# xin-fight/Research-and-Implementation-of-Image-Dehazing-Algorithm-Based-on-Vision-Transformer

Hardware: AMD Instinct MI355X
Metric: train patches/sec (128x128, embed_dim=32) (higher is better)
Workload: dtype f32; 1 GPU; Uformer_ProbSparse train step E=32 ps=128 per-GPU bs=32 fp32 Charbonnier+CR(VGG19, seeded-random weights) + AdamW (BASELINE configs[1]); global_batch=32, parallelism=dp1, arithmetic=fp32 storage/accumulate; products 6xbf16 MFMA, dropped <= 2^-24, split_terms=6

## Files before the change

### include/dehaze_hip.h

```cpp
#ifndef DEHAZE_HIP_H
#define DEHAZE_HIP_H

#include <stdint.h>

#ifdef __cplusplus
extern "C" {
#endif

#define DHZ_OK 0
#define DHZ_EINVAL (-22)
#define DHZ_ELAUNCH (-5)

#define DHZ_F32 0
#define DHZ_BF16 1

#define DHZ_NTOK 64
#define DHZ_NTOP 25

int dhz_abi_version(void);
const char* dhz_last_error(void);
const char* dhz_build_id(void);
int dhz_set_reserved_cus(int k);
int dhz_get_reserved_cus(void);
int dhz_grid_cus(void);
int dhz_set_deterministic(int on);
int dhz_get_deterministic(void);
int dhz_set_det_workspace(float* ws, size_t bytes);

int dhz_ps_attn_fwd(const float* q, const float* k, const float* v, int ld, const uint8_t* idx,
                    const float* bias, const float* mask, float* out, int ldo, uint8_t* rank,
                    int B_, int H, int nW, int d, void* stream);

int dhz_ps_attn_bwd_parts(int B_, int H);
int dhz_ps_attn_bwd_parts_d(int B_, int H, int d);
int dhz_ps_attn_bwd(const float* q, const float* k, const float* v, int ld, const float* bias,
                    const float* mask, const uint8_t* rank, const float* dout, int ldo, float* dq,
                    float* dk, float* dv, int ldg, float* dbias_part, int B_, int H, int nW, int d,
                    void* stream);

int dhz_fused_attn_prepack(const float* wq, const float* wk, const float* wv, const float* wo,
                           float* wqkv_p, float* wo_p, int C, void* stream);
int dhz_fused_attn_prepack_multi(const float* const* wq, const float* const* wk, const float* const* wv, const float* const* wo,
                                 float* const* wqkv_p, float* const* wo_p, const int* C, int n, void* stream);
int dhz_fused_window_attn_fwd(const float* x, const float* gamma, const float* beta, const float* wqkv_p,
                              const float* bqkv, const float* wo_p, const float* bo, const uint8_t* idx,
                              const float* bias, const float* mask, const float* drop_scale, float* out,
                              float* xn_save, float* qkv_save, float* ctx_save, float* stats_save,
                              uint8_t* rank_save, int B, int Hres, int Wres, int C, int shift,
                              void* stream);
int dhz_fused_window_attn_fwd6(const float* x, const float* gamma, const float* beta, const void* wqkv6_p, const float* bqkv,
                               const float* wo_p, const float* bo, const uint8_t* idx, const float* bias, const float* mask,
                               const float* drop_scale, float* out, float* xn_save, float* qkv_save, float* ctx_save, float* stats_save,
                               uint8_t* rank_save, int B, int Hres, int Wres, int C, int shift, void* stream);
// ... 304 lines not shown
```

### research-and-implementation-of-image-dehazing-algorithm-based-on-vision-transformer_amd/csrc/fused_attn.hip

```cpp
#include <stdlib.h>
#include "bf16_pipe.h"

namespace {

#ifndef FUSED_PERSIST_C32
#define FUSED_PERSIST_C32 1
#endif
#ifndef DHZ_FUSED_ABL
#define DHZ_FUSED_ABL 0
#endif
constexpr int NT = 64;
constexpr int NU = 25;
constexpr int SS = 68;
constexpr int HS = 36;

template <int CTRL>
__device__ __forceinline__ float dpp(float v) {
    return __int_as_float(__builtin_amdgcn_update_dpp(0, __float_as_int(v), CTRL, 0xF, 0xF, true));
}
__device__ __forceinline__ float r4max(float v) { v = fmaxf(v, dpp<0xB1>(v)); return fmaxf(v, dpp<0x4E>(v)); }
__device__ __forceinline__ float r4sum(float v) { v += dpp<0xB1>(v); return v + dpp<0x4E>(v); }
__device__ __forceinline__ float r8max(float v) { v = r4max(v); return fmaxf(v, dpp<0x141>(v)); }
__device__ __forceinline__ float r8sum(float v) { v = r4sum(v); return v + dpp<0x141>(v); }

// ... 20 lines not shown
    float vec[6 * C];
    int top[4][32];
    uint8_t idx[NT * NU];
};

template <int C, int SAVE, int NW = 1, bool P6 = false, bool PAD = false>
__global__ __launch_bounds__(256 * NW, NW == 2 ? 1 : (C == 64 ? 3 : (C == 128 ? 1 : 2))) void fused_window_attn_fwd_kernel(
    const float* __restrict__ x, const float* __restrict__ gamma, const float* __restrict__ beta,
    const float4* __restrict__ wqkv_p, const float* __restrict__ bqkv, const float4* __restrict__ wo_p,
    const float* __restrict__ bo, const uint8_t* __restrict__ idx, const float* __restrict__ bias,
    const float* __restrict__ mask, const float* __restrict__ dscale, float* __restrict__ out,
    float* __restrict__ xn_save, float* __restrict__ qkv_save, float* __restrict__ ctx_save,
    float* __restrict__ stats_save, uint8_t* __restrict__ rank_save, int Hres, int Wres, int shift, int nwin, PadArg<PAD> pad) {
    static_assert(!PAD || SAVE == 0, "padding words: inference instances only");
    constexpr int abl = DHZ_FUSED_ABL;
    constexpr int H = C / 32;
    constexpr int CPT = C / 4;
    constexpr int KS = C / 4;
    constexpr int KS4 = KS / 4;
    constexpr int P6_QKV_BYTES = (C / 32) * (C / 64 > 0 ? C / 64 : 1) * P6_RUNS * 1024;
    constexpr int P6O_RUNS = (C / 16) * 3;
    constexpr bool P6O = P6 && C >= 64 && P6O_RUNS * 1024 <= (int)sizeof(float) * NT * SS && P6O_RUNS % 4 == 0;
    extern __shared__ __attribute__((aligned(16))) unsigned char smem_raw[];
    const int half = NW == 2 ? (int)(threadIdx.x >> 8) : 0;
    FusedSmem<C>& sm = reinterpret_cast<FusedSmem<C>*>(smem_raw)[half];
    const int t = threadIdx.x & 255, lane = t & 63, w = t >> 6;
    const int i16 = lane & 15, g = lane >> 4;
    const int nWw = Wres >> 3, nW = (Hres >> 3) * nWw;
    const int tl = 16 * w + i16, qd = g;
    float* const P = sm.k;
// ... 58 lines not shown
            for (int i = 0; i < CPT / 4; ++i) {
                const float a0 = xv[i].x - mean, a1 = xv[i].y - mean, a2 = xv[i].z - mean, a3 = xv[i].w - mean;
                var += a0 * a0 + a1 * a1 + a2 * a2 + a3 * a3;
            }
            var = tok4sum(var);
            const float rstd = rsqrtf(var * (1.0f / C) + 1e-5f);
#pragma unroll
            for (int i = 0; i < CPT / 4; ++i) {
                const float4 gm = gmr[i], bt = btr[i];
                float4 y;
                y.x = (xv[i].x - mean) * rstd * gm.x + bt.x;
                y.y = (xv[i].y - mean) * rstd * gm.y + bt.y;
                y.z = (xv[i].z - mean) * rstd * gm.z + bt.z;
                y.w = (xv[i].w - mean) * rstd * gm.w + bt.w;
                xa[4 * i] = y.x; xa[4 * i + 1] = y.y; xa[4 * i + 2] = y.z; xa[4 * i + 3] = y.w;
                if (SAVE == 1 && !(abl & 128)) reinterpret_cast<float4*>(xn_save + ((size_t)win * NT + tl) * C + qd * CPT)[i] = y;
            }
            if (SAVE == 1 && !(abl & 128) && qd == 0) *reinterpret_cast<float2*>(stats_save + 2 * src_tok) = make_float2(mean, rstd);
        }
        dhz_u32x4 a6[P6 ? KS / 8 : 1][3];
        if constexpr (P6) {
#pragma unroll
            for (int kb = 0; kb < KS / 8; ++kb) dhz_split8x3(&xa[8 * kb], a6[kb][0], a6[kb][1], a6[kb][2]);
        }
        f32x4 oacc[C / 16];
#pragma unroll
        for (int i = 0; i < C / 16; ++i) oacc[i] = f32x4{0.f, 0.f, 0.f, 0.f};

#pragma unroll 1
        for (int h = 0; h < H; ++h) {
            if (!(abl & 1)) {
                const float (&a)[KS] = xa;
                f32x4 acc[6];
// ... 72 lines not shown
                        for (int j = 0; j < 6; ++j) acc[j] = mfma16(a[4 * s4 + 2], bc[j].z, acc[j]);
#pragma unroll
                        for (int j = 0; j < 6; ++j) acc[j] = mfma16(a[4 * s4 + 3], bc[j].w, acc[j]);
#pragma unroll
                        for (int j = 0; j < 6; ++j) bc[j] = bn[j];
                    }
                }
#pragma unroll
                for (int j = 0; j < 6; ++j) {
                    float* dst = (j < 2 ? sm.q : (j < 4 ? sm.k : sm.v)) + 16 * (j & 1) + i16;
#pragma unroll
                    for (int r = 0; r < 4; ++r) dst[(16 * w + 4 * g + r) * HS] = acc[j][r];
                }
            }
            __syncthreads();
            if (SAVE == 1 && !(abl & 128)) {
                const int row = t >> 2, c8 = (t & 3) * 8;
                float* dst = qkv_save + ((size_t)win * NT + row) * 3 * C + 32 * h + c8;
                *reinterpret_cast<float4*>(dst) = *reinterpret_cast<const float4*>(&sm.q[row * HS + c8]);
                *reinterpret_cast<float4*>(dst + 4) = *reinterpret_cast<const float4*>(&sm.q[row * HS + c8 + 4]);
                *reinterpret_cast<float4*>(dst + C) = *reinterpret_cast<const float4*>(&sm.k[row * HS + c8]);
                *reinterpret_cast<float4*>(dst + C + 4) = *reinterpret_cast<const float4*>(&sm.k[row * HS + c8 + 4]);
                *reinterpret_cast<float4*>(dst + 2 * C) = *reinterpret_cast<const float4*>(&sm.v[row * HS + c8]);
                *reinterpret_cast<float4*>(dst + 2 * C + 4) = *reinterpret_cast<const float4*>(&sm.v[row * HS + c8 + 4]);
            }
            if (!(abl & 2)) {
                float a[8], kb[4][8];
                f32x4 sacc[4];
                ld4(&sm.q[(16 * w + i16) * HS + 8 * g], &a[0]);
                ld4(&sm.q[(16 * w + i16) * HS + 8 * g + 4], &a[4]);
#pragma unroll
// ... 439 lines not shown
    DHZ_CHECK_LAUNCH("dhz_fused_attn_prepack_multi");
    return DHZ_OK;
}

static int fused_fwd_impl(bool p6, const float* x, const float* gamma, const float* beta, const float* wqkv_p,
                          const float* bqkv, const float* wo_p, const float* bo, const uint8_t* idx,
                          const float* bias, const float* mask, const float* drop_scale, float* out,
                          float* xn_save, float* qkv_save, float* ctx_save, float* stats_save,
                          uint8_t* rank_save, int B, int Hres, int Wres, int C, int shift, void* stream, const uint64_t* pad = nullptr) {
    DHZ_REQUIRE(x && gamma && beta && wqkv_p && bqkv && wo_p && bo && idx && out, "dhz_fused_window_attn_fwd: null pointer");
    DHZ_REQUIRE(C == 32 || C == 64 || C == 128, "dhz_fused_window_attn_fwd: C=%d unsupported (32, 64, 128)", C);
    DHZ_REQUIRE(B > 0 && Hres % 8 == 0 && Wres % 8 == 0 && Hres >= 8 && Wres >= 8 && shift >= 0 && shift < 8,
                "dhz_fused_window_attn_fwd: bad geometry %dx%d shift %d", Hres, Wres, shift);
    const bool any4 = xn_save || qkv_save || ctx_save || stats_save;
    const bool all4 = xn_save && qkv_save && ctx_save && stats_save;
    DHZ_REQUIRE(!any4 || (all4 && rank_save),
                "dhz_fused_window_attn_fwd: save buffers: none, rank_save alone, or all five");
    const int save = all4 ? 1 : (rank_save ? 2 : 0);
    DHZ_REQUIRE(!mask || shift > 0, "dhz_fused_window_attn_fwd: a mask is only meaningful for shifted windows");
    hipStream_t s = (hipStream_t)stream;
    const int nwin = B * (Hres / 8) * (Wres / 8);
#define GO(CC)                                                                                                      \
    do {                                                                                                            \
        if (save == 1) launch_fused<CC, 1>(s, nwin, x, gamma, beta, wqkv_p, bqkv, wo_p, bo, idx, bias, mask, drop_scale, \
                                           out, xn_save, qkv_save, ctx_save, stats_save, rank_save, Hres, Wres, shift);   \
        else if (save == 2) launch_fused<CC, 2>(s, nwin, x, gamma, beta, wqkv_p, bqkv, wo_p, bo, idx, bias, mask, drop_scale, \
                                                out, nullptr, nullptr, nullptr, nullptr, rank_save, Hres, Wres, shift);      \
        else if (pad) launch_fused<CC, 0, 1, false, true>(s, nwin, x, gamma, beta, wqkv_p, bqkv, wo_p, bo, idx, bias, mask, drop_scale, out, \
                                                          nullptr, nullptr, nullptr, nullptr, nullptr, Hres, Wres, shift, pad); \
        else launch_fused<CC, 0>(s, nwin, x, gamma, beta, wqkv_p, bqkv, wo_p, bo, idx, bias, mask, drop_scale, out, \
                                 nullptr, nullptr, nullptr, nullptr, nullptr, Hres, Wres, shift);                \
    } while (0)
#ifdef DHZ_DIAG
    static const int pair_env = getenv("DHZ_FUSED_PAIR") ? atoi(getenv("DHZ_FUSED_PAIR")) : 0;
#else
    constexpr int pair_env = 0;
#endif
    if (C == 64 && pair_env == 2 && nwin % 2 == 0 && !pad) {
        if (save == 1) launch_fused<64, 1, 2>(s, nwin, x, gamma, beta, wqkv_p, bqkv, wo_p, bo, idx, bias, mask, drop_scale, out, xn_save,
                                              qkv_save, ctx_save, stats_save, rank_save, Hres, Wres, shift);
        else if (save == 2) launch_fused<64, 2, 2>(s, nwin, x, gamma, beta, wqkv_p, bqkv, wo_p, bo, idx, bias, mask, drop_scale, out,
                                                   nullptr, nullptr, nullptr, nullptr, rank_save, Hres, Wres, shift);
        else launch_fused<64, 0, 2>(s, nwin, x, gamma, beta, wqkv_p, bqkv, wo_p, bo, idx, bias, mask, drop_scale, out, nullptr, nullptr,
                                    nullptr, nullptr, nullptr, Hres, Wres, shift);
    } else if (p6) {
        DHZ_REQUIRE(C == 32 || C == 64 || C == 128, "dhz_fused_window_attn_fwd6: C=%d unsupported (32, 64, 128)", C);
#define GO6(CC)                                                                                                             \
    do {                                                                                                                    \
        if (save == 1) launch_fused<CC, 1, 1, true>(s, nwin, x, gamma, beta, wqkv_p, bqkv, wo_p, bo, idx, bias, mask, drop_scale, out, xn_save, \
                                                    qkv_save, ctx_save, stats_save, rank_save, Hres, Wres, shift);         \
        else if (save == 2) launch_fused<CC, 2, 1, true>(s, nwin, x, gamma, beta, wqkv_p, bqkv, wo_p, bo, idx, bias, mask, drop_scale, out, \
                                                         nullptr, nullptr, nullptr, nullptr, rank_save, Hres, Wres, shift); \
        else if (pad) launch_fused<CC, 0, 1, true, true>(s, nwin, x, gamma, beta, wqkv_p, bqkv, wo_p, bo, idx, bias, mask, drop_scale, out, nullptr, \
                                                         nullptr, nullptr, nullptr, nullptr, Hres, Wres, shift, pad);      \
        else launch_fused<CC, 0, 1, true>(s, nwin, x, gamma, beta, wqkv_p, bqkv, wo_p, bo, idx, bias, mask, drop_scale, out, nullptr, nullptr, \
                                          nullptr, nullptr, nullptr, Hres, Wres, shift);                                   \
    } while (0)
        if (C == 32) GO6(32); else if (C == 64) GO6(64); else GO6(128);
#undef GO6
    } else if (C == 32) GO(32); else if (C == 64) GO(64); else GO(128);
#undef GO
    DHZ_CHECK_LAUNCH("dhz_fused_window_attn_fwd");
    return DHZ_OK;
}

extern "C" int dhz_fused_attn_prepack6_multi(const float* const* wq, const float* const* wk, const float* const* wv, const float* const* wo,
                                             void* const* wqkv6_p, const int* C, int n, void* stream) {
// ... 51 lines not shown
```

### research-and-implementation-of-image-dehazing-algorithm-based-on-vision-transformer_amd/csrc/ps_attn.hip

```cpp
#include "bf16_pipe.h"

namespace {

constexpr int NT = 64;
constexpr int NU = 25;
constexpr int SS = 68;

#ifndef PSF_WG32
#define PSF_WG32 3
#endif
#ifndef PSF_WG64
#define PSF_WG64 3
#endif

__device__ __forceinline__ dhz_bf16x8 frag_bf16(const float* row, int half, int g) {
    const f32x4 lo = *reinterpret_cast<const f32x4*>(row + 32 * half + 8 * g);
    const f32x4 hi = *reinterpret_cast<const f32x4*>(row + 32 * half + 8 * g + 4);
    dhz_u32x4 r;
    r[0] = dhz_pack_top(lo[1], lo[0]); r[1] = dhz_pack_top(lo[3], lo[2]);
    r[2] = dhz_pack_top(hi[1], hi[0]); r[3] = dhz_pack_top(hi[3], hi[2]);
    return __builtin_bit_cast(dhz_bf16x8, r);
}
__device__ __forceinline__ f32x4 tile_mma_bf16_k64(const float* A, int lda, const float* B, int ldb, int i16, int g, f32x4 acc) {
    acc = __builtin_amdgcn_mfma_f32_16x16x32_bf16(frag_bf16(A + i16 * lda, 0, g), frag_bf16(B + i16 * ldb, 0, g), acc, 0, 0, 0);
// ... 487 lines not shown
                if (r < NU) val = *reinterpret_cast<const float4*>(&dqs[r * DS + c4 * 4]);
                st4(dq + go, val);
            }
        }
    }

    if (HAS_BIAS && REG_ACC) {
        float* dst = dbias_part + (size_t)blockIdx.x * NT * NT;
#pragma unroll
        for (int i = 0; i < 16; ++i) dst[(w + 4 * i) * NT + lane] = accr[i];
    }
    if (HAS_BIAS && !REG_ACC) {
        __syncthreads();
        float4* dst = reinterpret_cast<float4*>(dbias_part + (size_t)blockIdx.x * NT * NT);
        for (int e = t; e < NT * NT / 4; e += 256) dst[e] = reinterpret_cast<const float4*>(sm.acc)[e];
    }
}

__global__ void bias_gather_kernel(const float* __restrict__ table, float* __restrict__ bias, int H) {
    const int e = blockIdx.x * blockDim.x + threadIdx.x;
    if (e >= H * NT * NT) return;
    const int h = e / (NT * NT), i = (e / NT) % NT, j = e % NT;
    const int rel = ((i >> 3) - (j >> 3) + 7) * 15 + ((i & 7) - (j & 7) + 7);
    bias[e] = table[rel * H + h];
}

constexpr int BIAS_MULTI_MAX = 32;
struct BiasMulti { const float* table[BIAS_MULTI_MAX]; float* bias[BIAS_MULTI_MAX]; int H[BIAS_MULTI_MAX]; };
__global__ void bias_gather_multi_kernel(const BiasMulti d) {
    const int H = d.H[blockIdx.y];
// ... 223 lines not shown
    dhz_set_error("dhz_ps_attn_bwd_dt: unknown dtype %d", dtype);
    return DHZ_EINVAL;
}
extern "C" int dhz_ps_attn_bwd_dt_pad(const void* q, const void* k, const void* v, int ld, const float* bias,
                                      const float* mask, const uint64_t* pad, const uint8_t* rank, const void* dout, int ldo, void* dq,
                                      void* dk, void* dv, int ldg, float* dbias_part, int B_, int H, int nW, int d,
                                      int dtype, void* stream) {
    DHZ_REQUIRE_PAD("dhz_ps_attn_bwd_dt_pad");
    if (dtype == DHZ_F32) return ps_attn_bwd_t<float>((const float*)q, (const float*)k, (const float*)v, ld, bias, mask, rank, (const float*)dout, ldo, (float*)dq, (float*)dk, (float*)dv, ldg, dbias_part, B_, H, nW, d, stream, pad);
    if (dtype == DHZ_BF16) return ps_attn_bwd_t<bf16s>((const bf16s*)q, (const bf16s*)k, (const bf16s*)v, ld, bias, mask, rank, (const bf16s*)dout, ldo, (bf16s*)dq, (bf16s*)dk, (bf16s*)dv, ldg, dbias_part, B_, H, nW, d, stream, pad);
    dhz_set_error("dhz_ps_attn_bwd_dt_pad: unknown dtype %d", dtype);
    return DHZ_EINVAL;
}
#undef DHZ_REQUIRE_PAD

extern "C" int dhz_bias_gather(const float* table, float* bias, int H, void* stream) {
    DHZ_REQUIRE(table && bias && H > 0, "dhz_bias_gather: bad arguments");
    const int n = H * NT * NT;
    hipLaunchKernelGGL(bias_gather_kernel, dim3((n + 255) / 256), dim3(256), 0, (hipStream_t)stream, table, bias, H);
    DHZ_CHECK_LAUNCH("dhz_bias_gather");
    return DHZ_OK;
}

extern "C" int dhz_bias_gather_multi(const float* const* tables, float* const* biases, const int* heads, int n, void* stream) {
    DHZ_REQUIRE(tables && biases && heads && n > 0 && n <= BIAS_MULTI_MAX, "dhz_bias_gather_multi: null pointer or n=%d outside 1..%d", n,
                BIAS_MULTI_MAX);
    BiasMulti d = {};
    int hmax = 0;
    for (int i = 0; i < n; ++i) {
        DHZ_REQUIRE(tables[i] && biases[i] && heads[i] > 0, "dhz_bias_gather_multi: entry %d: null pointer or H=%d", i, heads[i]);
// ... 63 lines not shown
```

### research-and-implementation-of-image-dehazing-algorithm-based-on-vision-transformer_amd/dehaze_hip/_lib.py

```python
import ctypes
import os

_HERE = os.path.dirname(os.path.abspath(__file__))
LIB_PATH = os.environ.get("DHZ_LIB_PATH") or os.path.join(_HERE, "libdehaze_hip.so")

c_f = ctypes.c_void_p
c_p = ctypes.c_void_p
c_i = ctypes.c_int
c_l = ctypes.c_int64
c_fl = ctypes.c_float

SIGNATURES = {
    "dhz_abi_version": [],
    "dhz_last_error": [],
    "dhz_build_id": [],
    "dhz_set_reserved_cus": [ctypes.c_int],
    "dhz_gelu_fwd_dt": [ctypes.c_void_p, ctypes.c_void_p, ctypes.c_int64, ctypes.c_int, ctypes.c_void_p],
    "dhz_gelu_bwd_dt": [ctypes.c_void_p, ctypes.c_void_p, ctypes.c_void_p, ctypes.c_int64, ctypes.c_void_p, ctypes.c_int64, ctypes.c_int, ctypes.c_void_p],
    "dhz_get_reserved_cus": [],
    "dhz_set_deterministic": [ctypes.c_int],
    "dhz_get_deterministic": [],
    "dhz_set_det_workspace": [ctypes.c_void_p, ctypes.c_size_t],
    "dhz_grid_cus": [],
    "dhz_ps_attn_fwd": [c_f, c_f, c_f, c_i, c_p, c_f, c_f, c_f, c_i, c_p, c_i, c_i, c_i, c_i, c_p],
    "dhz_ps_attn_bwd_parts": [c_i, c_i],
    "dhz_ps_attn_bwd_parts_d": [c_i, c_i, c_i],
    "dhz_ps_attn_bwd": [c_f, c_f, c_f, c_i, c_f, c_f, c_p, c_f, c_i, c_f, c_f, c_f, c_i, c_f, c_i, c_i, c_i, c_i, c_p],
    "dhz_fused_attn_prepack": [c_f, c_f, c_f, c_f, c_f, c_f, c_i, c_p],
    "dhz_fused_window_attn_fwd": [c_f, c_f, c_f, c_f, c_f, c_f, c_f, c_p, c_f, c_f, c_f, c_f, c_f, c_f, c_f, c_f, c_p,
                                  c_i, c_i, c_i, c_i, c_i, c_p],
    "dhz_fused_window_attn_fwd6": [c_f, c_f, c_f, c_f, c_f, c_f, c_f, c_p, c_f, c_f, c_f, c_f, c_f, c_f, c_f, c_f, c_p,
                                   c_i, c_i, c_i, c_i, c_i, c_p],
    "dhz_fused_attn_prepack6": [c_f, c_f, c_f, c_f, c_p, c_i, c_p],
    "dhz_fused_attn_prepack6_multi": [c_p, c_p, c_p, c_p, c_p, c_p, c_i, c_p],
    "dhz_fused_attn_bwd_parts": [c_i],
    "dhz_fused_attn_bwd_prepack": [c_f, c_f, c_f, c_f, c_f, c_i, c_p],
    "dhz_fused_window_attn_bwd": [c_f] * 11 + [c_f] * 12 + [c_i, c_i, c_i, c_i, c_i, c_p],
    "dhz_dense_attn_fwd": [c_f, c_f, c_f, c_i, c_f, c_f, c_f, c_i, c_i, c_i, c_i, c_i, c_fl, c_p],
    "dhz_dense_attn_bwd": [c_f, c_f, c_f, c_i, c_f, c_f, c_f, c_i, c_f, c_f, c_f, c_i, c_f, c_i, c_i, c_i, c_i, c_fl, c_p],
    "dhz_bias_gather": [c_f, c_f, c_i, c_p],
    "dhz_bias_gather_multi": [c_p, c_p, c_p, c_i, c_p],
    "dhz_fused_attn_prepack_multi": [c_p, c_p, c_p, c_p, c_p, c_p, c_p, c_i, c_p],
# ... 172 lines not shown
```

### research-and-implementation-of-image-dehazing-algorithm-based-on-vision-transformer_amd/dehaze_hip/fused.py

```python
import torch
from torch.autograd import Function

from . import _lib, ops
from .ops import NTOK, _grad_buf, _int_array, _p, _ptr_array, _ready, _require_gpu, _stream

SUPPORTED_C = (32, 64, 128)
ENABLED = True
ATTN_FUSED_C128_MAX_HW = int(__import__("os").environ.get("DHZ_FUSED_C128_MAX_HW", "1024"))
ATTN_FUSED_BWD_C = (32,)


def _fused_bwd_widths():
    return () if ops.DETERMINISTIC else ATTN_FUSED_BWD_C
ATTN_FUSED_P6 = __import__("os").environ.get("DHZ_FUSED_P6", "1") != "0"
ATTN_FUSED_P6_C = (64, 128)
ATTN_FUSED_PAD_P6_C = (64, 128)
LEFF_FUSED = True
LEFF_FUSED_C = (32, 64)
LEFF_FUSED_C64_MAX_T = 262144
LEFF_FUSED_P6 = __import__("os").environ.get("DHZ_LEFF_P6", "1") != "0"
LEFF_FUSED_P6_C = (64,)
LEFF_BWD_DZ = __import__("os").environ.get("DHZ_LEFF_BWD_DZ", "1") != "0"
LEFF_BWD_DZ_C = (32, 64, 128)


def _wgrad(dy, off, x, w, b, row_scale=None):
    return ops.linear_wgrad(dy, off, x, [(w, b)], row_scale)


def _ln_backward(dxn, x, gamma_p, beta_p, gamma, stats, dres, B, Hres, Wres, C, shift, partition, dres_windowed=False, dx_window=None,
                 dx2=None):
    dx = torch.empty_like(x)
    gg, gb = _grad_buf(gamma_p), _grad_buf(beta_p)
    lay = (1 if dres_windowed else 0, 0 if dx_window is None else 1, 0 if dx_window is None else int(dx_window))
    d2 = None
    if dx2 is not None:
        d2 = torch.empty_like(x)
        lay = (lay[0], lay[1], int(dx2[0]))
# ... 154 lines not shown
            _lib.call("dhz_fused_attn_prepack", _p(wq), _p(wk), _p(wv), _p(wo), _p(wqkv_p), _p(wo_p), C, _stream())
    wqkv_f32 = wqkv_p
    if use6:
        hit = STAGED_PACK6.pop(id(wq), None)
        if hit is not None and hit[0] is wq and hit[1].numel() == n6 and hit[1].device == dev:
            wqkv_p = hit[1]
        else:
            wqkv_p = torch.empty(n6, device=dev, dtype=torch.bfloat16)
            _lib.call("dhz_fused_attn_prepack6", _p(wq), _p(wk), _p(wv), _p(wo), _p(wqkv_p), C, _stream())
        if wo_p is None:
            wo_p = wqkv_p
    bqkv = ops.cat_rows([bq.detach(), bk.detach(), bv.detach()])
    bias = _bias_tile(table, H, dev)
    out = torch.empty_like(x)
    fused_bwd = train and C in _fused_bwd_widths() and x.dtype == torch.float32
    xn = qkv = cx = stats = rank = None
    if train:
        if not fused_bwd:
            xn = torch.empty((T, C), **f32)
            qkv = torch.empty((T, 3 * C), **f32)
            cx = torch.empty((T, C), **f32)
            stats = torch.empty((T, 2), **f32)
        rank = torch.empty(((T // NTOK) * H * NTOK,), device=dev, dtype=torch.uint8)
    entry = "dhz_fused_window_attn_fwd6" if use6 else "dhz_fused_window_attn_fwd"
    ev = ops._timed("dhz_fused_window_attn_fwd")
    if pad is not None:
        assert pad.is_cuda and pad.dtype == torch.int64 and pad.numel() == T // NTOK and pad.is_contiguous(), \
            f"padding words {tuple(pad.shape)} {pad.dtype} on {pad.device}"
        _lib.call("dhz_fused_window_attn_fwd_pad", 1 if use6 else 0, _p(x), _p(gamma), _p(beta), _p(wqkv_p), _p(bqkv), _p(wo_p), _p(bo), _p(idx),
                  _p(bias), _p(mask), _p(pad), _p(dscale), _p(out), B, Hres, Wres, C, shift, _stream())
    else:
        _lib.call(entry, _p(x), _p(gamma), _p(beta), _p(wqkv_p), _p(bqkv), _p(wo_p), _p(bo), _p(idx),
                  _p(bias), _p(mask), _p(dscale), _p(out), _p(xn), _p(qkv), _p(cx), _p(stats), _p(rank), B, Hres, Wres, C,
                  shift, _stream())
    ops._timed_end(ev, T // NTOK, C)
    rec = None
# ... 62 lines not shown


def _attn_bwd(rec, dout, windowed=False, daw_pre=None):
    if rec.kind == "attn_fused_bwd":
        assert not windowed
        return _attn_bwd_fused(rec, dout)
    x, gamma, stats, xn, qkv, cx, rank, bias, mask, dscale, wq_, wk_, wv_, wo_ = rec.saved
    wq, bq, wk, bk, wv, bv, wo, bo, gamma_p, beta_p, table_p = rec.params
    B, Hres, Wres, C, shift, H = rec.geom
    d = C // H
    dout = dout.contiguous()
    dev = x.device
    T = B * Hres * Wres
    B_ = T // NTOK
    f32 = dict(device=dev, dtype=torch.float32)
    if daw_pre is not None:
        daw = daw_pre.view(T, C)
        dctx = ops.gemm_dgrad(daw, wo_)
        g_wo, g_bo = _wgrad(daw, 0, cx, wo, bo)
    elif windowed:
        daw = dout.view(T, C)
        rs = (dscale, Hres * Wres) if dscale is not None else None
        dctx = ops.gemm_dgrad(daw, wo_, rs)
        g_wo, g_bo = _wgrad(daw, 0, cx, wo, bo, rs)
    else:
        daw = torch.empty((T, C), device=dev, dtype=dout.dtype)
        _lib.call("dhz_reverse_residual_bwd_dt", _p(dout), _p(dscale), _p(daw), B, Hres, Wres, C, shift, 1, ops._dt(dout), _stream())
        dctx = ops.gemm_dgrad(daw, wo_)
        g_wo, g_bo = _wgrad(daw, 0, cx, wo, bo)
    dqkv = torch.empty_like(qkv)
    parts = _lib.load().dhz_ps_attn_bwd_parts_d(B_, H, d)
    dpart = torch.empty((parts, NTOK, NTOK), **f32) if bias is not None else None
    ops.ps_attn_bwd_launch(qkv, dqkv, bias, mask, rank, dctx, dpart, B_, H, d)
    dtable = _table_backward(dpart, parts, table_p, H, dev) if bias is not None else None
    dxn, (g_wq, g_bq, g_wk, g_bk, g_wv, g_bv) = ops.linear_bwd_pair(dqkv, xn, ops.cat_rows([wq_.detach(), wk_.detach(), wv_.detach()]),
                                                                    [(wq, bq), (wk, bk), (wv, bv)])
    dx, dgamma, dbeta = _ln_backward(dxn, x, gamma_p, beta_p, gamma, stats, dout, B, Hres, Wres, C, shift, 1, dres_windowed=windowed)
    return (dx, dgamma, dbeta, g_wq, g_bq, g_wk, g_bk, g_wv, g_bv, g_wo, g_bo, dtable)


def fused_c128_ok(HW):
    return HW <= ATTN_FUSED_C128_MAX_HW or not torch.is_grad_enabled()


def use_fused_attn(C, dtype, heads, HW):
    return ENABLED and dtype == torch.float32 and C == 32 * heads and (C in (32, 64) or (C == 128 and fused_c128_ok(HW)))


# ... 261 lines not shown
```

Before: 1034 patches/s.

## Fuse attention out-projection backward into ProbSparse attention backward kernel

Adds a ProbSparse attention backward kernel that also does the out-projection backward. It computes dctx from daw and Wo inside the kernel, accumulates dWo/dbo with fp32 atomics, and exploits the rank structure so that only the top rows plus one mean row of daw are needed. The forward then no longer saves the ctx buffer for C=64 (new save mode 3). This removes a separate dgrad GEMM, a wgrad GEMM and a T×C ctx write and read. The trade-offs are atomic contention on the weight gradients, no support for deterministic mode, and the path only runs for C=64 layers.

```diff
diff --git a/include/dehaze_hip.h b/include/dehaze_hip.h
--- a/include/dehaze_hip.h
+++ b/include/dehaze_hip.h
@@ -37,6 +37,11 @@
                     const float* mask, const uint8_t* rank, const float* dout, int ldo, float* dq,
                     float* dk, float* dv, int ldg, float* dbias_part, int B_, int H, int nW, int d,
                     void* stream);
+
+int dhz_ps_attn_bwd_outproj(const float* q, const float* k, const float* v, int ld, const float* bias, const float* mask,
+                            const uint8_t* rank, const float* daw, int lda, const float* wo, const float* row_scale, int wins_per_scale,
+                            float* dq, float* dk, float* dv, int ldg, float* dbias_part, float* dwo, float* dbo, int B_, int H, int nW,
+                            int d, void* stream);
 
 int dhz_fused_attn_prepack(const float* wq, const float* wk, const float* wv, const float* wo,
                            float* wqkv_p, float* wo_p, int C, void* stream);
diff --git a/research-and-implementation-of-image-dehazing-algorithm-based-on-vision-transformer_amd/csrc/fused_attn.hip b/research-and-implementation-of-image-dehazing-algorithm-based-on-vision-transformer_amd/csrc/fused_attn.hip
--- a/research-and-implementation-of-image-dehazing-algorithm-based-on-vision-transformer_amd/csrc/fused_attn.hip
+++ b/research-and-implementation-of-image-dehazing-algorithm-based-on-vision-transformer_amd/csrc/fused_attn.hip
@@ -58,6 +58,7 @@
     float* __restrict__ stats_save, uint8_t* __restrict__ rank_save, int Hres, int Wres, int shift, int nwin, PadArg<PAD> pad) {
     static_assert(!PAD || SAVE == 0, "padding words: inference instances only");
     constexpr int abl = DHZ_FUSED_ABL;
+    constexpr bool SAVE_CHAIN = SAVE == 1 || SAVE == 3;
     constexpr int H = C / 32;
     constexpr int CPT = C / 4;
     constexpr int KS = C / 4;
@@ -146,9 +147,9 @@
                 y.z = (xv[i].z - mean) * rstd * gm.z + bt.z;
                 y.w = (xv[i].w - mean) * rstd * gm.w + bt.w;
                 xa[4 * i] = y.x; xa[4 * i + 1] = y.y; xa[4 * i + 2] = y.z; xa[4 * i + 3] = y.w;
-                if (SAVE == 1 && !(abl & 128)) reinterpret_cast<float4*>(xn_save + ((size_t)win * NT + tl) * C + qd * CPT)[i] = y;
-            }
-            if (SAVE == 1 && !(abl & 128) && qd == 0) *reinterpret_cast<float2*>(stats_save + 2 * src_tok) = make_float2(mean, rstd);
+                if (SAVE_CHAIN && !(abl & 128)) reinterpret_cast<float4*>(xn_save + ((size_t)win * NT + tl) * C + qd * CPT)[i] = y;
+            }
+            if (SAVE_CHAIN && !(abl & 128) && qd == 0) *reinterpret_cast<float2*>(stats_save + 2 * src_tok) = make_float2(mean, rstd);
         }
         dhz_u32x4 a6[P6 ? KS / 8 : 1][3];
         if constexpr (P6) {
@@ -251,7 +252,7 @@
                 }
             }
             __syncthreads();
-            if (SAVE == 1 && !(abl & 128)) {
+            if (SAVE_CHAIN && !(abl & 128)) {
                 const int row = t >> 2, c8 = (t & 3) * 8;
                 float* dst = qkv_save + ((size_t)win * NT + row) * 3 * C + 32 * h + c8;
                 *reinterpret_cast<float4*>(dst) = *reinterpret_cast<const float4*>(&sm.q[row * HS + c8]);
@@ -721,9 +722,10 @@
                 "dhz_fused_window_attn_fwd: bad geometry %dx%d shift %d", Hres, Wres, shift);
     const bool any4 = xn_save || qkv_save || ctx_save || stats_save;
     const bool all4 = xn_save && qkv_save && ctx_save && stats_save;
-    DHZ_REQUIRE(!any4 || (all4 && rank_save),
-                "dhz_fused_window_attn_fwd: save buffers: none, rank_save alone, or all five");
-    const int save = all4 ? 1 : (rank_save ? 2 : 0);
+    const bool no_ctx = xn_save && qkv_save && !ctx_save && stats_save && C != 32;
+    DHZ_REQUIRE(!any4 || ((all4 || no_ctx) && rank_save),
+                "dhz_fused_window_attn_fwd: save buffers: none, rank_save alone, all five, or (C = 64 / 128) all but ctx_save");
+    const int save = all4 ? 1 : (no_ctx ? 3 : (rank_save ? 2 : 0));
     DHZ_REQUIRE(!mask || shift > 0, "dhz_fused_window_attn_fwd: a mask is only meaningful for shifted windows");
     hipStream_t s = (hipStream_t)stream;
     const int nwin = B * (Hres / 8) * (Wres / 8);
@@ -733,6 +735,8 @@
                                            out, xn_save, qkv_save, ctx_save, stats_save, rank_save, Hres, Wres, shift);   \
         else if (save == 2) launch_fused<CC, 2>(s, nwin, x, gamma, beta, wqkv_p, bqkv, wo_p, bo, idx, bias, mask, drop_scale, \
                                                 out, nullptr, nullptr, nullptr, nullptr, rank_save, Hres, Wres, shift);      \
+        else if (save == 3) { if constexpr (CC != 32) launch_fused<CC, 3>(s, nwin, x, gamma, beta, wqkv_p, bqkv, wo_p, bo, idx, bias, mask, drop_scale, \
+                                                out, xn_save, qkv_save, nullptr, stats_save, rank_save, Hres, Wres, shift); }  \
         else if (pad) launch_fused<CC, 0, 1, false, true>(s, nwin, x, gamma, beta, wqkv_p, bqkv, wo_p, bo, idx, bias, mask, drop_scale, out, \
                                                           nullptr, nullptr, nullptr, nullptr, nullptr, Hres, Wres, shift, pad); \
         else launch_fused<CC, 0>(s, nwin, x, gamma, beta, wqkv_p, bqkv, wo_p, bo, idx, bias, mask, drop_scale, out, \
@@ -743,7 +747,7 @@
 #else
     constexpr int pair_env = 0;
 #endif
-    if (C == 64 && pair_env == 2 && nwin % 2 == 0 && !pad) {
+    if (C == 64 && pair_env == 2 && nwin % 2 == 0 && !pad && save != 3) {
         if (save == 1) launch_fused<64, 1, 2>(s, nwin, x, gamma, beta, wqkv_p, bqkv, wo_p, bo, idx, bias, mask, drop_scale, out, xn_save,
                                               qkv_save, ctx_save, stats_save, rank_save, Hres, Wres, shift);
         else if (save == 2) launch_fused<64, 2, 2>(s, nwin, x, gamma, beta, wqkv_p, bqkv, wo_p, bo, idx, bias, mask, drop_scale, out,
@@ -758,6 +762,8 @@
                                                     qkv_save, ctx_save, stats_save, rank_save, Hres, Wres, shift);         \
         else if (save == 2) launch_fused<CC, 2, 1, true>(s, nwin, x, gamma, beta, wqkv_p, bqkv, wo_p, bo, idx, bias, mask, drop_scale, out, \
                                                          nullptr, nullptr, nullptr, nullptr, rank_save, Hres, Wres, shift); \
+        else if (save == 3) { if constexpr (CC != 32) launch_fused<CC, 3, 1, true>(s, nwin, x, gamma, beta, wqkv_p, bqkv, wo_p, bo, idx, bias, mask, drop_scale, out, \
+                                                         xn_save, qkv_save, nullptr, stats_save, rank_save, Hres, Wres, shift); } \
         else if (pad) launch_fused<CC, 0, 1, true, true>(s, nwin, x, gamma, beta, wqkv_p, bqkv, wo_p, bo, idx, bias, mask, drop_scale, out, nullptr, \
                                                          nullptr, nullptr, nullptr, nullptr, Hres, Wres, shift, pad);      \
         else launch_fused<CC, 0, 1, true>(s, nwin, x, gamma, beta, wqkv_p, bqkv, wo_p, bo, idx, bias, mask, drop_scale, out, nullptr, nullptr, \
diff --git a/research-and-implementation-of-image-dehazing-algorithm-based-on-vision-transformer_amd/csrc/ps_attn.hip b/research-and-implementation-of-image-dehazing-algorithm-based-on-vision-transformer_amd/csrc/ps_attn.hip
--- a/research-and-implementation-of-image-dehazing-algorithm-based-on-vision-transformer_amd/csrc/ps_attn.hip
+++ b/research-and-implementation-of-image-dehazing-algorithm-based-on-vision-transformer_amd/csrc/ps_attn.hip
@@ -525,6 +525,280 @@
         __syncthreads();
         float4* dst = reinterpret_cast<float4*>(dbias_part + (size_t)blockIdx.x * NT * NT);
         for (int e = t; e < NT * NT / 4; e += 256) dst[e] = reinterpret_cast<const float4*>(sm.acc)[e];
+    }
+}
+
+template <int C>
+struct OutprojSmem {
+    static constexpr int CS = C + 4;
+    BwdSmem<32> core;
+    float tile[32 * CS];
+};
+static_assert(sizeof(BwdSmem<32>) % 16 == 0, "the daw tile starts 16-byte aligned");
+
+template <int C, bool HAS_BIAS>
+__global__ __launch_bounds__(256) void ps_attn_bwd_outproj_kernel(
+    const float* __restrict__ q, const float* __restrict__ k, const float* __restrict__ v, int ld,
+    const float* __restrict__ bias, const float* __restrict__ mask, const uint8_t* __restrict__ rank_in,
+    const float* __restrict__ daw, int lda, const float* __restrict__ wo, const float* __restrict__ row_scale, int wins_per_scale,
+    float* __restrict__ dq, float* __restrict__ dk, float* __restrict__ dv, int ldg, float* __restrict__ dbias_part,
+    float* __restrict__ dwo, float* __restrict__ dbo, int B_, int nW) {
+    constexpr int D = 32, H = C / 32;
+    constexpr int DS = D + 4, CS = C + 4;
+    constexpr int F = D / 4, RPP = 256 / F, NR = NT / RPP;
+    constexpr int FC = C / 4, RC = 256 / FC, NRC = NT / RC;
+    constexpr int NW = C / 32;
+    extern __shared__ __attribute__((aligned(16))) unsigned char smem_raw[];
+    OutprojSmem<C>& so = *reinterpret_cast<OutprojSmem<C>*>(smem_raw);
+    BwdSmem<D>& sm = so.core;
+    float* const tile = so.tile;
+    const int t = threadIdx.x, lane = t & 63, w = t >> 6;
+    const int i16 = lane & 15, g = lane >> 4;
+    const int bid = blockIdx.x;
+    const int h = bid % H;
+    const int bstep = gridDim.x / H;
+    const float scale = rsqrtf((float)D);
+    const int tr = w & 1, tc2 = w >> 1;
+
+    if (HAS_BIAS) {
+        for (int e = t; e < NT * NT / 4; e += 256) reinterpret_cast<float4*>(sm.acc)[e] = make_float4(0.f, 0.f, 0.f, 0.f);
+    }
+    float wf[C / 4];
+#pragma unroll
+    for (int s = 0; s < C / 4; ++s) wf[s] = wo[(size_t)(4 * s + g) * C + 32 * h + 16 * tc2 + i16];
+    f32x4 accw[NW];
+#pragma unroll
+    for (int ii = 0; ii < NW; ++ii) accw[ii] = f32x4{0.f, 0.f, 0.f, 0.f};
+    float dbacc = 0.f;
+
+    f32x4 pk[NR], pv[NR], pq[NR], pg[NRC];
+    uint8_t prank = 255;
+    auto prefetch = [&](int b) {
+        const size_t tok0 = (size_t)b * NT;
+        const int c4 = t % F;
+#pragma unroll
+        for (int p = 0; p < NR; ++p) {
+            const size_t gi = (tok0 + p * RPP + t / F) * ld + h * D + c4 * 4;
+            pk[p] = ld4v(k + gi);
+            pv[p] = ld4v(v + gi);
+            pq[p] = ld4v(q + gi);
+        }
+#pragma unroll
+        for (int p = 0; p < NRC; ++p) pg[p] = ld4v(daw + (tok0 + p * RC + t / FC) * lda + (t % FC) * 4);
+        if (t < NT) prank = rank_in[((size_t)b * H + h) * NT + t];
+    };
+    if (bid / H < B_) prefetch(bid / H);
+
+    for (int b = bid / H; b < B_; b += bstep) {
+        const size_t tok0 = (size_t)b * NT;
+        const float rs = row_scale ? row_scale[b / wins_per_scale] : 1.0f;
+        __syncthreads();
+        if (t < NT) {
+            const uint8_t r = prank;
+            sm.rank[t] = r;
+            if (r < NU) sm.top[r] = t;
+        } else if (t < NT + 32 - NU) {
+            sm.top[NU + t - NT] = 0;
+        }
+        for (int e = t; e < (32 - NU) * DS; e += 256) sm.qr[NU * DS + e] = 0.f;
+        for (int e = t; e < (31 - NU) * CS; e += 256) tile[(NU + 1) * CS + e] = 0.f;
+        __syncthreads();
+
+        {
+            const int c4 = t % F;
+#pragma unroll
+            for (int p = 0; p < NR; ++p) {
+                const int row = p * RPP + t / F;
+                *reinterpret_cast<f32x4*>(&sm.k[row * DS + c4 * 4]) = pk[p];
+                *reinterpret_cast<f32x4*>(&sm.v[row * DS + c4 * 4]) = pv[p];
+                const int r = sm.rank[row];
+                if (r < NU) *reinterpret_cast<f32x4*>(&sm.qr[r * DS + c4 * 4]) = pq[p];
+            }
+            const int cc = t % FC;
+            f32x4 dm = {0.f, 0.f, 0.f, 0.f};
+#pragma unroll
+            for (int p = 0; p < NRC; ++p) {
+                const int r = sm.rank[p * RC + t / FC];
+                const f32x4 val = pg[p] * rs;
+                if (r < NU) *reinterpret_cast<f32x4*>(&tile[r * CS + cc * 4]) = val;
+                else dm += val;
+            }
+            if (b + bstep < B_) prefetch(b + bstep);
+#pragma unroll
+            for (int o = FC; o < 64; o <<= 1) {
+                dm[0] += __shfl_xor(dm[0], o); dm[1] += __shfl_xor(dm[1], o);
+                dm[2] += __shfl_xor(dm[2], o); dm[3] += __shfl_xor(dm[3], o);
+            }
+            if (lane < FC) *reinterpret_cast<f32x4*>(&sm.ds[w * C + lane * 4]) = dm;
+        }
+        __syncthreads();
+        if (t < C) tile[NU * CS + t] = sm.ds[t] + sm.ds[C + t] + sm.ds[2 * C + t] + sm.ds[3 * C + t];
+
+        {
+#pragma unroll
+            for (int ii = 0; ii < 2; ++ii) {
+                const int tc = (w >> 1) + 2 * ii;
+                f32x4 acc = {0.f, 0.f, 0.f, 0.f};
+                acc = tile_mma<D / 4>(sm.qr + 16 * tr * DS, DS, 1, sm.k + 16 * tc * DS, DS, 1, acc);
+#pragma unroll
+                for (int j = 0; j < 4; ++j) sm.p1[(16 * tr + 4 * g + j) * SS + 16 * tc + i16] = acc[j];
+            }
+        }
+        __syncthreads();
+
+        {
+            f32x4 acc = {0.f, 0.f, 0.f, 0.f};
+            const float* ap = tile + (16 * tr + i16) * CS + g;
+#pragma unroll
+            for (int s = 0; s < C / 4; ++s) acc = mfma16(ap[4 * s], wf[s], acc);
+#pragma unroll
+            for (int j = 0; j < 4; ++j) sm.dor[(16 * tr + 4 * g + j) * DS + 16 * tc2 + i16] = acc[j];
+        }
+        {
+            const int r = t >> 3, c0 = (t & 7) * 8;
+            float p1[8], p2[8];
+            if (r < NU) {
+                const int qrow = sm.top[r];
+                float x[8];
+#pragma unroll
+                for (int i = 0; i < 8; ++i) x[i] = sm.p1[r * SS + c0 + i] * scale;
+                const float* brow = bias ? bias + ((size_t)h * NT + qrow) * NT + c0 : nullptr;
+                const float* mrow = mask ? mask + ((size_t)(b % nW) * NT + qrow) * NT + c0 : nullptr;
+                double_softmax8<false>(x, brow, mrow, p1, p2);
+            } else {
+                const float f = (r == NU) ? (1.0f / NT) : 0.f;
+#pragma unroll
+                for (int i = 0; i < 8; ++i) { p1[i] = 0.f; p2[i] = f; }
+            }
+#pragma unroll
+            for (int i = 0; i < 8; ++i) { sm.p1[r * SS + c0 + i] = p1[i]; sm.p2[r * SS + c0 + i] = p2[i]; }
+        }
+        __syncthreads();
+
+        f32x4 accv[D / 16];
+        f32x4 accp[2];
+        f32x4 acco = {0.f, 0.f, 0.f, 0.f};
+        {
+#pragma unroll
+            for (int tc = 0; tc < D / 16; ++tc) {
+                f32x4 acc = {0.f, 0.f, 0.f, 0.f};
+                accv[tc] = tile_mma<8>(sm.p2 + 16 * w, 1, SS, sm.dor + 16 * tc, 1, DS, acc);
+            }
+#pragma unroll
+            for (int ii = 0; ii < 2; ++ii) {
+                const int tc = (w >> 1) + 2 * ii;
+                f32x4 acc = {0.f, 0.f, 0.f, 0.f};
+                accp[ii] = tile_mma<D / 4>(sm.dor + 16 * tr * DS, DS, 1, sm.v + 16 * tc * DS, DS, 1, acc);
+            }
+            acco = tile_mma<16>(sm.p2 + 16 * tr * SS, SS, 1, sm.v + 16 * tc2, 1, DS, acco);
+        }
+        __syncthreads();
+        {
+#pragma unroll
+            for (int tc = 0; tc < D / 16; ++tc)
+#pragma unroll
+                for (int j = 0; j < 4; ++j) sm.v[(16 * w + 4 * g + j) * DS + 16 * tc + i16] = accv[tc][j];
+#pragma unroll
+            for (int ii = 0; ii < 2; ++ii) {
+                const int tc = (w >> 1) + 2 * ii;
+#pragma unroll
+                for (int j = 0; j < 4; ++j) sm.ds[(16 * tr + 4 * g + j) * SS + 16 * tc + i16] = accp[ii][j];
+            }
+#pragma unroll
+            for (int j = 0; j < 4; ++j) sm.dor[(16 * tr + 4 * g + j) * DS + 16 * tc2 + i16] = acco[j];
+        }
+        __syncthreads();
+
+        {
+            const int r = t >> 3, c0 = (t & 7) * 8;
+            float dp[8], p1[8], p2[8];
+            float dot2 = 0.f;
+#pragma unroll
+            for (int i = 0; i < 8; ++i) {
+                dp[i] = sm.ds[r * SS + c0 + i]; p1[i] = sm.p1[r * SS + c0 + i]; p2[i] = sm.p2[r * SS + c0 + i];
+                dot2 += dp[i] * p2[i];
+            }
+            dot2 = dhz_row8_sum(dot2);
+            float da[8], dot1 = 0.f;
+#pragma unroll
+            for (int i = 0; i < 8; ++i) { da[i] = p2[i] * (dp[i] - dot2); dot1 += da[i] * p1[i]; }
+            dot1 = dhz_row8_sum(dot1);
+            if (HAS_BIAS && r < NU) {
+                float* arow = sm.acc + sm.top[r] * NT + c0;
+#pragma unroll
+                for (int i = 0; i < 8; ++i) arow[i] += da[i];
+            }
+#pragma unroll
+            for (int i = 0; i < 8; ++i) sm.ds[r * SS + c0 + i] = p1[i] * (da[i] - dot1) * scale;
+
+            const int c4 = t % F;
+#pragma unroll
+            for (int p = 0; p < NR; ++p) {
+                const int row = p * RPP + t / F;
+                st4(dv + (tok0 + row) * ldg + h * D + c4 * 4, *reinterpret_cast<const float4*>(&sm.v[row * DS + c4 * 4]));
+            }
+        }
+        __syncthreads();
+
+        f32x4 accq;
+        f32x4 acck[D / 16];
+        {
+            f32x4 acc = {0.f, 0.f, 0.f, 0.f};
+            accq = tile_mma<16>(sm.ds + 16 * tr * SS, SS, 1, sm.k + 16 * tc2, 1, DS, acc);
+#pragma unroll
+            for (int tc = 0; tc < D / 16; ++tc) {
+                f32x4 a2 = {0.f, 0.f, 0.f, 0.f};
+                acck[tc] = tile_mma<8>(sm.ds + 16 * w, 1, SS, sm.qr + 16 * tc, 1, DS, a2);
+            }
+#pragma unroll
+            for (int ii = 0; ii < NW; ++ii) accw[ii] = tile_mma<8>(tile + 16 * (tc2 + 2 * ii), 1, CS, sm.dor + 16 * tr, 1, DS, accw[ii]);
+            if (t < D) {
+                float su = 0.f;
+#pragma unroll
+                for (int r = 0; r <= NU; ++r) su += tile[r * CS + 32 * h + t];
+                dbacc += su;
+            }
+        }
+        __syncthreads();
+        {
+            float* dqs = sm.p1;
+#pragma unroll
+            for (int j = 0; j < 4; ++j) dqs[(16 * tr + 4 * g + j) * DS + 16 * tc2 + i16] = accq[j];
+#pragma unroll
+            for (int tc = 0; tc < D / 16; ++tc)
+#pragma unroll
+                for (int j = 0; j < 4; ++j) sm.k[(16 * w + 4 * g + j) * DS + 16 * tc + i16] = acck[tc][j];
+        }
+        __syncthreads();
+        {
+            const float* dqs = sm.p1;
+            const int c4 = t % F;
+#pragma unroll
+            for (int p = 0; p < NR; ++p) {
+                const int row = p * RPP + t / F;
+                const size_t go = (tok0 + row) * ldg + h * D + c4 * 4;
+                st4(dk + go, *reinterpret_cast<const float4*>(&sm.k[row * DS + c4 * 4]));
+                const int r = sm.rank[row];
+                float4 val = make_float4(0.f, 0.f, 0.f, 0.f);
+                if (r < NU) val = *reinterpret_cast<const float4*>(&dqs[r * DS + c4 * 4]);
+                st4(dq + go, val);
+            }
+        }
+    }
+
+    __syncthreads();
+    if (HAS_BIAS) {
+        float4* dst = reinterpret_cast<float4*>(dbias_part + (size_t)bid * NT * NT);
+        for (int e = t; e < NT * NT / 4; e += 256) dst[e] = reinterpret_cast<const float4*>(sm.acc)[e];
+    }
+    if (bid / H < B_) {
+#pragma unroll
+        for (int ii = 0; ii < NW; ++ii)
+#pragma unroll
+            for (int j = 0; j < 4; ++j) tile[(16 * (tc2 + 2 * ii) + 4 * g + j) * D + 16 * tr + i16] = accw[ii][j];
+        __syncthreads();
+        for (int e = t; e < C * D; e += 256) atomicAdd(dwo + (size_t)(e / D) * C + 32 * h + e % D, tile[e]);
+        if (t < D) atomicAdd(dbo + 32 * h + t, dbacc);
     }
 }
 
@@ -778,6 +1052,53 @@
 }
 #undef DHZ_REQUIRE_PAD
 
+template <int C, bool HB>
+static void launch_bwd_outproj(int parts, hipStream_t s, const float* q, const float* k, const float* v, int ld, const float* bias,
+                               const float* mask, const uint8_t* rank, const float* daw, int lda, const float* wo, const float* row_scale,
+                               int wins_per_scale, float* dq, float* dk, float* dv, int ldg, float* dbias_part, float* dwo, float* dbo,
+                               int B_, int nW) {
+    const size_t smem = sizeof(OutprojSmem<C>);
+    dhz_allow_smem(&ps_attn_bwd_outproj_kernel<C, HB>, smem);
+    hipLaunchKernelGGL((ps_attn_bwd_outproj_kernel<C, HB>), dim3(parts), dim3(256), smem, s, q, k, v, ld, bias, mask, rank, daw, lda, wo,
+                       row_scale, wins_per_scale, dq, dk, dv, ldg, dbias_part, dwo, dbo, B_, nW);
+}
+
+extern "C" int dhz_ps_attn_bwd_outproj(const float* q, const float* k, const float* v, int ld, const float* bias, const float* mask,
+                                       const uint8_t* rank, const float* daw, int lda, const float* wo, const float* row_scale,
+                                       int wins_per_scale, float* dq, float* dk, float* dv, int ldg, float* dbias_part, float* dwo,
+                                       float* dbo, int B_, int H, int nW, int d, void* stream) {
+    const char* who = "dhz_ps_attn_bwd_outproj";
+    DHZ_REQUIRE(!dhz_det(), "%s: accumulates dWo / dbo with fp32 atomics: not available in deterministic mode (run the out-projection's "
+                            "backward products and dhz_ps_attn_bwd)", who);
+    DHZ_REQUIRE(q && k && v && rank && daw && wo && dq && dk && dv && dwo && dbo, "%s: null pointer", who);
+    DHZ_REQUIRE(d == 32 && (H == 2 || H == 4), "%s: head_dim %d, %d heads: instances are head_dim 32 with 2 or 4 heads (C = 64, 128)", who, d, H);
+    DHZ_REQUIRE(B_ > 0, "%s: B_=%d", who, B_);
+    const int C = H * d;
+    DHZ_REQUIRE(!bias || dbias_part, "%s: bias given but dbias_part is NULL", who);
+    DHZ_REQUIRE(ld % 4 == 0 && ldg % 4 == 0 && ld >= C && ldg >= C, "%s: ld=%d / ldg=%d must be multiples of 4 and at least C=%d", who, ld, ldg, C);
+    DHZ_REQUIRE(lda % 4 == 0 && lda >= C, "%s: lda=%d must be a multiple of 4 and at least C=%d", who, lda, C);
+    DHZ_REQUIRE(!(((uintptr_t)q | (uintptr_t)k | (uintptr_t)v | (uintptr_t)daw | (uintptr_t)dq | (uintptr_t)dk | (uintptr_t)dv) & 15),
+                "%s: q, k, v, daw, dq, dk, dv must be 16-byte aligned", who);
+    DHZ_REQUIRE(!mask || (nW > 0 && B_ % nW == 0), "%s: B_=%d not a multiple of nW=%d", who, B_, nW);
+    DHZ_REQUIRE(!row_scale || (wins_per_scale > 0 && B_ % wins_per_scale == 0), "%s: B_=%d is not a whole number of images of %d windows", who,
+                B_, wins_per_scale);
+    hipStream_t s = (hipStream_t)stream;
+    const int parts = dhz_ps_attn_bwd_parts_d(B_, H, d);
+    if (nW <= 0) nW = 1;
+    if (!row_scale) wins_per_scale = 1;
+#define GO(CC)                                                                                                                     \
+    do {                                                                                                                           \
+        if (bias) launch_bwd_outproj<CC, true>(parts, s, q, k, v, ld, bias, mask, rank, daw, lda, wo, row_scale, wins_per_scale, dq, dk, dv, \
+                                               ldg, dbias_part, dwo, dbo, B_, nW);                                            \
+        else launch_bwd_outproj<CC, false>(parts, s, q, k, v, ld, bias, mask, rank, daw, lda, wo, row_scale, wins_per_scale, dq, dk, dv, \
+                                           ldg, dbias_part, dwo, dbo, B_, nW);                                                \
+    } while (0)
+    if (H == 2) GO(64); else GO(128);
+#undef GO
+    DHZ_CHECK_LAUNCH(who);
+    return DHZ_OK;
+}
+
 extern "C" int dhz_bias_gather(const float* table, float* bias, int H, void* stream) {
     DHZ_REQUIRE(table && bias && H > 0, "dhz_bias_gather: bad arguments");
     const int n = H * NT * NT;
diff --git a/research-and-implementation-of-image-dehazing-algorithm-based-on-vision-transformer_amd/dehaze_hip/_lib.py b/research-and-implementation-of-image-dehazing-algorithm-based-on-vision-transformer_amd/dehaze_hip/_lib.py
--- a/research-and-implementation-of-image-dehazing-algorithm-based-on-vision-transformer_amd/dehaze_hip/_lib.py
+++ b/research-and-implementation-of-image-dehazing-algorithm-based-on-vision-transformer_amd/dehaze_hip/_lib.py
@@ -26,6 +26,8 @@
     "dhz_ps_attn_bwd_parts": [c_i, c_i],
     "dhz_ps_attn_bwd_parts_d": [c_i, c_i, c_i],
     "dhz_ps_attn_bwd": [c_f, c_f, c_f, c_i, c_f, c_f, c_p, c_f, c_i, c_f, c_f, c_f, c_i, c_f, c_i, c_i, c_i, c_i, c_p],
+    "dhz_ps_attn_bwd_outproj": [c_f, c_f, c_f, c_i, c_f, c_f, c_p, c_f, c_i, c_f, c_f, c_i, c_f, c_f, c_f, c_i, c_f, c_f, c_f, c_i, c_i,
+                                c_i, c_i, c_p],
     "dhz_fused_attn_prepack": [c_f, c_f, c_f, c_f, c_f, c_f, c_i, c_p],
     "dhz_fused_window_attn_fwd": [c_f, c_f, c_f, c_f, c_f, c_f, c_f, c_p, c_f, c_f, c_f, c_f, c_f, c_f, c_f, c_f, c_p,
                                   c_i, c_i, c_i, c_i, c_i, c_p],
diff --git a/research-and-implementation-of-image-dehazing-algorithm-based-on-vision-transformer_amd/dehaze_hip/fused.py b/research-and-implementation-of-image-dehazing-algorithm-based-on-vision-transformer_amd/dehaze_hip/fused.py
--- a/research-and-implementation-of-image-dehazing-algorithm-based-on-vision-transformer_amd/dehaze_hip/fused.py
+++ b/research-and-implementation-of-image-dehazing-algorithm-based-on-vision-transformer_amd/dehaze_hip/fused.py
@@ -22,6 +22,15 @@
 LEFF_FUSED_P6_C = (64,)
 LEFF_BWD_DZ = __import__("os").environ.get("DHZ_LEFF_BWD_DZ", "1") != "0"
 LEFF_BWD_DZ_C = (32, 64, 128)
+ATTN_BWD_OUTPROJ = __import__("os").environ.get("DHZ_ATTN_BWD_OUTPROJ", "1") != "0"
+ATTN_BWD_OUTPROJ_BUILT = (64, 128)
+ATTN_BWD_OUTPROJ_C = (64,)
+
+
+def attn_bwd_outproj_ok(C, dtype, wo, bo, head_dim=32, win=8, pad=False):
+    if not ATTN_BWD_OUTPROJ or C not in ATTN_BWD_OUTPROJ_C or head_dim != 32 or ops.DETERMINISTIC or dtype != torch.float32 or win != 8 or pad:
+        return False
+    return all(p is not None and p.is_leaf and p.requires_grad and (p.grad is None or p.grad.is_contiguous()) for p in (wo, bo))
 
 
 def _wgrad(dy, off, x, w, b, row_scale=None):
@@ -206,12 +215,13 @@
     bias = _bias_tile(table, H, dev)
     out = torch.empty_like(x)
     fused_bwd = train and C in _fused_bwd_widths() and x.dtype == torch.float32
+    no_cx = train and not fused_bwd and attn_bwd_outproj_ok(C, x.dtype, wo, bo, pad=pad is not None)
     xn = qkv = cx = stats = rank = None
     if train:
         if not fused_bwd:
             xn = torch.empty((T, C), **f32)
             qkv = torch.empty((T, 3 * C), **f32)
-            cx = torch.empty((T, C), **f32)
+            cx = None if no_cx else torch.empty((T, C), **f32)
             stats = torch.empty((T, 2), **f32)
         rank = torch.empty(((T // NTOK) * H * NTOK,), device=dev, dtype=torch.uint8)
     entry = "dhz_fused_window_attn_fwd6" if use6 else "dhz_fused_window_attn_fwd"
@@ -304,24 +314,38 @@
     T = B * Hres * Wres
     B_ = T // NTOK
     f32 = dict(device=dev, dtype=torch.float32)
+    outproj = daw_pre is None and dout.dtype == torch.float32 and attn_bwd_outproj_ok(C, qkv.dtype, wo, bo, head_dim=d)
+    if cx is None and not outproj:
+        raise RuntimeError("dehaze_hip: the attention forward saved no ctx (its backward was to run dhz_ps_attn_bwd_outproj) and the backward "
+                           "cannot take that kernel any more: requires_grad of the out-projection, the deterministic mode or "
+                           "fused.ATTN_BWD_OUTPROJ changed between forward and backward")
+    rs = None
     if daw_pre is not None:
         daw = daw_pre.view(T, C)
-        dctx = ops.gemm_dgrad(daw, wo_)
-        g_wo, g_bo = _wgrad(daw, 0, cx, wo, bo)
     elif windowed:
         daw = dout.view(T, C)
         rs = (dscale, Hres * Wres) if dscale is not None else None
-        dctx = ops.gemm_dgrad(daw, wo_, rs)
-        g_wo, g_bo = _wgrad(daw, 0, cx, wo, bo, rs)
     else:
         daw = torch.empty((T, C), device=dev, dtype=dout.dtype)
         _lib.call("dhz_reverse_residual_bwd_dt", _p(dout), _p(dscale), _p(daw), B, Hres, Wres, C, shift, 1, ops._dt(dout), _stream())
-        dctx = ops.gemm_dgrad(daw, wo_)
-        g_wo, g_bo = _wgrad(daw, 0, cx, wo, bo)
+    if not outproj:
+        dctx = ops.gemm_dgrad(daw, wo_, rs)
+        g_wo, g_bo = _wgrad(daw, 0, cx, wo, bo, rs)
     dqkv = torch.empty_like(qkv)
     parts = _lib.load().dhz_ps_attn_bwd_parts_d(B_, H, d)
     dpart = torch.empty((parts, NTOK, NTOK), **f32) if bias is not None else None
-    ops.ps_attn_bwd_launch(qkv, dqkv, bias, mask, rank, dctx, dpart, B_, H, d)
+    if outproj:
+        gwo, gbo = ops._grad_pair(wo, bo)
+        if _p(daw) % 16:
+            daw = daw.clone()
+        base, gb = qkv.data_ptr(), dqkv.data_ptr()
+        _lib.call("dhz_ps_attn_bwd_outproj", base, base + 4 * C, base + 8 * C, 3 * C, _p(bias), _p(mask), _p(rank), _p(daw), daw.stride(0),
+                  _p(wo_ if wo_.is_contiguous() else wo_.contiguous()), _p(rs[0]) if rs else None, rs[1] // NTOK if rs else 0,
+                  gb, gb + 4 * C, gb + 8 * C, 3 * C, _p(dpart), _p(gwo), _p(gbo), B_, H, mask.shape[0] if mask is not None else 1, d, _stream())
+        _ready(wo, bo)
+        g_wo = g_bo = None
+    else:
+        ops.ps_attn_bwd_launch(qkv, dqkv, bias, mask, rank, dctx, dpart, B_, H, d)
     dtable = _table_backward(dpart, parts, table_p, H, dev) if bias is not None else None
     dxn, (g_wq, g_bq, g_wk, g_bk, g_wv, g_bv) = ops.linear_bwd_pair(dqkv, xn, ops.cat_rows([wq_.detach(), wk_.detach(), wv_.detach()]),
                                                                     [(wq, bq), (wk, bk), (wv, bv)])
```

Result: no change. 1042 patches/s (median of 6 runs) (+0.8%).
